# Tani843/Mixed_Precision_Multigrid_Solvers_for_PDEs

Measured on AMD Instinct MI355X. Metric: MDoF/s per V-cycle on 2D Poisson, higher is better.
Workload: dtype f64 (adaptive policy); 1 GPU; 2D Poisson 4097^2 adaptive fp32->fp64 (switch_threshold=1e-6), V(2,2) weighted-Jacobi omega=0.8, 11 levels, 1xMI355X; levels=11, cycle=V(2,2), smoother=jacobi, parallelism=1 GPU

## Files before the change

mixed_precision_multigrid_solvers_for_pdes_amd/csrc/mg_host.hpp:

```cpp
#pragma once

#include <hip/hip_runtime.h>

#include <cmath>
#include <cstdlib>
#include <string>
#include <vector>

#include "../../include/mghip.h"
#include "mg_kernels.hpp"

namespace mgh {

inline size_t esize(int dt) { return dt == MG_F32 ? 4 : 8; }
inline bool valid_dtype(int dt) { return dt == MG_F32 || dt == MG_F64; }

struct Coef {
  double ihx2, ihy2, diag, invD;
  bool pow2;
  bool all_pow2;
};
inline Coef coefs(double hx, double hy, double sigma = 0.0) {
  Coef c;
  c.ihx2 = 1.0 / (hx * hx);
// ... 54 lines not shown
  int* h_int = nullptr;
  mg::HostMailbox* mbox = nullptr;
  mg::HostMailbox* mbox_dev = nullptr;
  unsigned long long mbox_seq = 0;
  void* staging = nullptr;
  int grid_dtype = MG_F64;
  int phase = MG_F64;
  bool promoted = false;
  double fp32_floor = 0.0;
  int switch_reason = 0;
  bool have_rhs = false;
  bool varcoef = false;
  double sigma = 0.0;
  double rd_sigma = -1.0;
  double ring_sumsq[2] = {0, 0};
  unsigned rhs_gen = 1;
  unsigned rings_gen[2] = {0, 0};
  bool iterate_zero = false;
  unsigned zero_norm_gen[2] = {0, 0};
  double zero_norm_val[2] = {0, 0};
  int norm_partials = 0;
  int tail_start = -1;
  bool span_ring[2] = {false, false};
  int tail2_start = -1;
  int tail2_ntop = 0;
  int* d_tail_ops = nullptr;
  int tail_nops = 0;
  bool tail_direct = false;
  double tail_minv[81] = {0};
  double* d_minv = nullptr;
  int minv_n = 0;
  double tail_minv_sigma = -1.0;
  std::string err;
  std::vector<double> adapt_hist;

  int L() const { return (int)lv.size(); }
  int level_dtype_in(int l, int ph) const {
    if (l == L() - 1) return grid_dtype;
    switch (cfg.precision) {
      case MG_PREC_SINGLE: return MG_F32;
      case MG_PREC_SINGLE_MANAGED: return MG_F32;
      case MG_PREC_DEFECT: return MG_F32;
      case MG_PREC_MIXED_LEVELS: return (l >= (cfg.mixed_split > 0 ? cfg.mixed_split : L() / 2)) ? MG_F32 : MG_F64;
      case MG_PREC_ADAPTIVE: return ph;
      default: return MG_F64;
    }
// ... 17 lines not shown
```

mixed_precision_multigrid_solvers_for_pdes_amd/csrc/mg_kernels.hpp:

```cpp
#pragma once

#include <hip/hip_runtime.h>
#include <stdint.h>
#include <type_traits>

namespace mg {

constexpr int kBlock = 256;
constexpr int kTileRowBytes = 512;
constexpr int kTI = 32;
constexpr int kNumXcd = 8;
constexpr int kCoarseTag = 0, kFineTag = 1;
constexpr int kSmJacobi = 0, kSmRbgs = 1;
__host__ __device__ constexpr int sweep_halo(int sm) { return sm == kSmRbgs ? 2 : 1; }

template <typename T> struct VecW { static constexpr int N = 16 / sizeof(T); };

template <typename T> struct alignas(16) Pack {
  T v[VecW<T>::N];
};

template <typename T> __device__ __forceinline__ Pack<T> ldg(const T* p) {
  return *reinterpret_cast<const Pack<T>*>(p);
}
// ... 166 lines not shown
  }
  {
    const int lo = __double2loint(x), hi = __double2hiint(x);
    x += __hiloint2double(__builtin_amdgcn_permlane16_swap(hi, hi, false, false)[1],
                          __builtin_amdgcn_permlane16_swap(lo, lo, false, false)[1]);
  }
  x += dpp_row_move<0x108>(x);
  x += dpp_row_move<0x104>(x);
  x += dpp_row_move<0x102>(x);
  x += dpp_row_move<0x101>(x);
  return x;
}
__device__ __forceinline__ double row0_reduce_sum(double x) {
  x += dpp_row_move<0x108>(x);
  x += dpp_row_move<0x104>(x);
  x += dpp_row_move<0x102>(x);
  x += dpp_row_move<0x101>(x);
  return x;
}
__device__ __forceinline__ double wave_first(double x) {
  return __hiloint2double(__builtin_amdgcn_readfirstlane(__double2hiint(x)), __builtin_amdgcn_readfirstlane(__double2loint(x)));
}

template <int NW = kBlock / 64>
__device__ __forceinline__ double block_reduce_sum(double x, double* red) {
  x = wave_reduce_sum(x);
  const int lane = threadIdx.x & 63, wid = threadIdx.x >> 6;
  if (lane == 0) red[wid] = x;
  __syncthreads();
  double t = 0.0;
  if (threadIdx.x == 0) {
#pragma unroll
    for (int w = 0; w < NW; ++w) t += red[w];
  }
  return t;
}

template <typename T, bool WRITE_R, bool NORM, int TAG>
__global__ __launch_bounds__(kBlock) void residual_kernel(const T* __restrict__ u, const T* __restrict__ rhs,
                                                          T* __restrict__ r, double* __restrict__ partials, TileGeom g,
                                                          T ihx2, T ihy2, T diag, T coeff) {
  using S = TileShape<T>;
  __shared__ __attribute__((aligned(16))) T s[S::LDS_ELEMS];
  __shared__ double red[kBlock / 64];
  const int L = xcd_remap(blockIdx.x, g.ntiles);
  const int ti = L / g.tiles_j, tj = L - ti * g.tiles_j;
  const int i0 = g.i_org + ti * kTI, j0 = tj * S::TJ;
  const int cg = threadIdx.x % S::CG, rg = threadIdx.x / S::CG;
  const int gj0 = j0 + cg * S::N;
  const int lr = rg * S::RPT;

  Pack<T> f[S::RPT];
// ... 1536 lines not shown
```

mixed_precision_multigrid_solvers_for_pdes_amd/csrc/mg_rb_kernels.hpp:

```cpp
#pragma once

#include "mg_kernels.hpp"

namespace mg {

#ifndef MG_RB_HL_MIN
#define MG_RB_HL_MIN 4
#endif
template <typename T, int HALO, int W, int RPT> struct RbShape {
  static constexpr int N = VecW<T>::N;
  static constexpr int HL = (MG_RB_HL_MIN <= 2 && 2 * N >= HALO) ? 2 : ((HALO + N - 1) / N > 4 ? (HALO + N - 1) / N : 4);
  static constexpr int RI = W * RPT;
  static constexpr int RJ = 64 * N;
  static constexpr int TI = RI - 2 * HALO;
  static constexpr int TJ = (64 - 2 * HL) * N;
  static_assert(TI > 0 && TI % 2 == 0, "tile height must be even (coarse rows sit on every other tile row)");
  static_assert(RPT % 2 == 0, "rows per wave must be even (row parities are compile-time constants per strip row)");
  static_assert(HL * N >= HALO, "lateral halo too narrow");
};

#ifndef MG_RB_NT_MODE
#define MG_RB_NT_MODE 3
#endif
template <typename T> __device__ __forceinline__ T dpp_from_lower_lane(T x);
// ... 49 lines not shown
    const f2 sx0 = f2{dn.v[0], dn.v[1]} + f2{up.v[0], up.v[1]}, sx1 = f2{dn.v[2], dn.v[3]} + f2{up.v[2], up.v[3]};
    const f2 sy0 = f2{mid.v[1], mid.v[2]} + f2{left, mid.v[0]}, sy1 = f2{mid.v[3], right} + f2{mid.v[1], mid.v[2]};
    const f2 nb0 = ihx2 * sx0 + ihy2 * sy0, nb1 = ihx2 * sx1 + ihy2 * sy1;
    const f2 t0 = f2{f.v[0], f.v[1]} + nb0, t1 = f2{f.v[2], f.v[3]} + nb1;
    const f2 un0 = use_div ? t0 / D : t0 * invD, un1 = use_div ? t1 / D : t1 * invD;
    const f2 r0 = one_m_omega * m0 + omega * un0, r1 = one_m_omega * m1 + omega * un1;
    Pack<float> res;
    res.v[0] = r0.x; res.v[1] = r0.y; res.v[2] = r1.x; res.v[3] = r1.y;
    return res;
  }
  static __device__ __forceinline__ Pack<float> resid(const Pack<float>& mid, const Pack<float>& dn, const Pack<float>& up, float left,
                                                      float right, const Pack<float>& f, float ihx2, float ihy2, float D, float coeff) {
    const f2 m0 = {mid.v[0], mid.v[1]}, m1 = {mid.v[2], mid.v[3]};
    const f2 sx0 = f2{dn.v[0], dn.v[1]} + f2{up.v[0], up.v[1]}, sx1 = f2{dn.v[2], dn.v[3]} + f2{up.v[2], up.v[3]};
    const f2 sy0 = f2{mid.v[1], mid.v[2]} + f2{left, mid.v[0]}, sy1 = f2{mid.v[3], right} + f2{mid.v[1], mid.v[2]};
    const f2 au0 = coeff * ((sx0 * ihx2 + sy0 * ihy2) - m0 * D), au1 = coeff * ((sx1 * ihx2 + sy1 * ihy2) - m1 * D);
    const f2 r0 = f2{f.v[0], f.v[1]} - au0, r1 = f2{f.v[2], f.v[3]} - au1;
    Pack<float> r;
    r.v[0] = r0.x; r.v[1] = r0.y; r.v[2] = r1.x; r.v[3] = r1.y;
    return r;
  }
};

template <typename T, int W>
__device__ __forceinline__ void rb_exchange(Pack<T>* __restrict__ xb, int w, int lane, const Pack<T>& top, const Pack<T>& bottom,
                                            Pack<T>& above, Pack<T>& below) {
  xb[(w * 2 + 0) * 64 + lane] = top;
  xb[(w * 2 + 1) * 64 + lane] = bottom;
  __syncthreads();
  above = (w > 0) ? xb[((w - 1) * 2 + 1) * 64 + lane] : zero_pack<T>();
  below = (w < W - 1) ? xb[((w + 1) * 2 + 0) * 64 + lane] : zero_pack<T>();
}

template <typename T, int HALO, bool PROLONG, int POST, bool ZERO_INIT, typename TX, typename TC, int SM, int W, int RPT, bool INT, int NT,
          bool VAR, int SPAN = 0>
__device__ __forceinline__ void rb_leg_body(const T* __restrict__ u, const T* __restrict__ rhs, T* __restrict__ out,
                                            const TX* __restrict__ e_coarse, TX* __restrict__ rhs_coarse,
                                            double* __restrict__ partials, const FusedArgs& a, T ihx2, T ihy2, T invD, T D, T omega,
                                            T one_m_omega, T coeff, Pack<T>* __restrict__ xbuf, TX* __restrict__ patch,
                                            double* __restrict__ red, int i0, int j0, const T* __restrict__ acoef, T sigma,
                                            const T* __restrict__ rdiag, T* __restrict__ out2 = nullptr) {
  static_assert(SPAN == 0 || (PROLONG && POST == kPostRestrict && !ZERO_INIT), "a spanning leg is an up leg followed by a down leg");
  using S = RbShape<T, HALO, W, RPT>;
  constexpr int N = S::N;
  constexpr int PH = S::RI / 2 + 2, PW = S::RJ / 2 + 2;
  constexpr int kRowPar = (1 - HALO) & 1;
  const int ri0 = i0 - HALO, rj0 = j0 - S::HL * N;
  const int lane = threadIdx.x & 63, w = __builtin_amdgcn_readfirstlane(threadIdx.x >> 6);
  const int gj0 = rj0 + lane * N;
  const int r_base = w * RPT;
  const bool col_in = INT || (gj0 >= 0 && gj0 < a.nyv);

  const int pic0 = (ri0 >> 1) + a.ci_off, pjc0 = (rj0 >> 1) + a.cj_off;
  if (PROLONG) {
    for (int idx = threadIdx.x; idx < PH * PW; idx += W * 64) {
      const int pr = idx / PW, pc = idx - pr * PW;
      const int ic = pic0 + pr, jc = pjc0 + pc;
      patch[idx] = (INT || (ic >= 0 && ic < a.nxc && jc >= 0 && jc < a.nyc)) ? e_coarse[(size_t)ic * a.ldc + jc] : TX(0);
    }
  }
  Pack<T> F[RPT], U[RPT];
#pragma unroll
  for (int k = 0; k < RPT; ++k) {
    const int gi = ri0 + r_base + k;
    F[k] = zero_pack<T>();
    U[k] = zero_pack<T>();
    if (INT || (gi >= 0 && gi < a.nx && col_in)) {
      F[k] = (NT & 4) ? ldg_nt(rhs + (size_t)gi * a.ld + gj0) : ldg(rhs + (size_t)gi * a.ld + gj0);
      if (!ZERO_INIT) U[k] = (NT & 2) ? ldg_nt(u + (size_t)gi * a.ld + gj0) : ldg(u + (size_t)gi * a.ld + gj0);
    }
  }
  constexpr int AVK = VAR ? RPT + 1 : 1, AHK = VAR ? RPT : 1, AHN = VAR ? N + 1 : 1;
  Pack<T> av[AVK];
  T ah[AHK][AHN];
  Pack<T> RD[AHK];
  if (VAR) {
    Pack<T> A[RPT];
#pragma unroll
    for (int k = 0; k < RPT; ++k) {
      const int gi = ri0 + r_base + k;
      A[k] = zero_pack<T>();
      RD[VAR ? k : 0] = zero_pack<T>();
      if (INT || (gi >= 0 && gi < a.nx && col_in)) {
        A[k] = ldg(acoef + (size_t)gi * a.ld + gj0);
        RD[VAR ? k : 0] = ldg(rdiag + (size_t)gi * a.ld + gj0);
      }
    }
    Pack<T> a_above, a_below;
    rb_exchange<T, W>(xbuf + (size_t)W * 2 * 64, w, lane, A[0], A[RPT - 1], a_above, a_below);
#pragma unroll
    for (int k = 0; k < RPT; ++k) {
      const Pack<T> up = (k > 0) ? A[k > 0 ? k - 1 : 0] : a_above;
      const Pack<T> dn = (k < RPT - 1) ? A[k < RPT - 1 ? k + 1 : 0] : a_below;
      const T left = dpp_from_lower_lane<T>(A[k].v[N - 1]);
      const T right = dpp_from_upper_lane<T>(A[k].v[0]);
#pragma unroll
      for (int e = 0; e < N; ++e) {
        av[VAR ? k : 0].v[e] = T(0.5) * (A[k].v[e] + up.v[e]);
        if (k == RPT - 1) av[VAR ? RPT : 0].v[e] = T(0.5) * (A[k].v[e] + dn.v[e]);
        ah[VAR ? k : 0][VAR ? e : 0] = T(0.5) * (A[k].v[e] + ((e == 0) ? left : A[k].v[e > 0 ? e - 1 : 0]));
      }
      ah[VAR ? k : 0][VAR ? N : 0] = T(0.5) * (A[k].v[N - 1] + right);
    }
  }
  if (PROLONG) {
    __syncthreads();
    using TS = typename std::conditional<(sizeof(TC) > sizeof(T)), TC, T>::type;
    if (INT) {
      constexpr int M = N / 2 + 1;
      const TX* pl = patch + (r_base / 2) * PW + lane * (N / 2);
#pragma unroll
      for (int k = 0; k < RPT; ++k) {
        const bool iodd = ((kRowPar + k) & 1) != 0;
        const int pr = (k + kRowPar) >> 1;
        TC av[M], bv[M];
#pragma unroll
        for (int m = 0; m < M; ++m) {
          av[m] = (TC)pl[pr * PW + m];
          bv[m] = iodd ? (TC)pl[(pr + 1) * PW + m] : TC(0);
        }
#pragma unroll
        for (int e = 0; e < N; ++e) {
          const int m = e >> 1;
          TC val;
          if ((e & 1) == 0) val = iodd ? TC(0.5) * (av[m] + bv[m]) : av[m];
          else val = iodd ? TC(0.25) * (((av[m] + av[m + 1]) + bv[m]) + bv[m + 1]) : TC(0.5) * (av[m] + av[m + 1]);
          U[k].v[e] = (T)((TS)U[k].v[e] + (TS)val);
        }
      }
    } else {
      const TX* pe = patch - ((ptrdiff_t)pic0 * PW + pjc0);
#pragma unroll
      for (int k = 0; k < RPT; ++k) {
        const int gi = ri0 + r_base + k;
        if (gi >= 0 && gi < a.nx && col_in) {
          TC val[N];
          bool ok[N];
          prolong_vec<TX, TC, N>(pe, PW, a.nxc, a.nyc, gi, gj0, a.nx, a.ny, a.sides, val, ok, a.ci_off, a.cj_off);
#pragma unroll
          for (int e = 0; e < N; ++e)
            if (ok[e]) U[k].v[e] = (T)((TS)U[k].v[e] + (TS)val[e]);
        }
      }
    }
  }

  int stage = 0;
  auto run_sweeps = [&](int nsw) {
  const int npass = (SM == kSmRbgs) ? 2 * nsw : nsw;
  for (int s = 0; s < npass; ++s, ++stage) {
    Pack<T> above, below;
    rb_exchange<T, W>(xbuf + (size_t)(stage & 1) * W * 2 * 64, w, lane, U[0], U[RPT - 1], above, below);
    const int colour = s & 1;
    static_assert(N % 2 == 0 && RPT % 2 == 0, "strip rows / lane cells must be even for a workgroup-uniform colour parity");
    const int par0 = (ri0 + rj0 + a.colour_offset) & 1;
    auto pass = [&](auto qp) {
      constexpr int QP = decltype(qp)::value;
      Pack<T> prev = above;
#pragma unroll
      for (int k = 0; k < RPT; ++k) {
        const int r = r_base + k, gi = ri0 + r;
        const Pack<T> mid = U[k];
        const Pack<T> dn = (k < RPT - 1) ? U[k + 1] : below;
        const T left = dpp_from_lower_lane<T>(mid.v[N - 1]);
        const T right = dpp_from_upper_lane<T>(mid.v[0]);
        Pack<T> o = mid;
        const bool row_ok = INT ? ((k > 0 || w > 0) && (k < RPT - 1 || w < W - 1))
                                : (r >= 1 && r < S::RI - 1 && gi >= 1 && gi < a.nx - 1);
        if (row_ok && !VAR) {
          const Pack<T> res = RowMath<T, N>::relax(mid, dn, prev, left, right, F[k], ihx2, ihy2, invD, D, omega, one_m_omega, a.use_div != 0);
#pragma unroll
          for (int e = 0; e < N; ++e) {
            const int gj = gj0 + e;
            const bool mine = (SM != kSmRbgs) || (((QP + k + e) & 1) == 0);
            if ((INT || (gj >= 1 && gj < a.ny - 1)) && mine) o.v[e] = res.v[e];
// ... 22 lines not shown
    else pass(std::integral_constant<int, 0>{});
  }
  };
  run_sweeps(a.nsweep);

  const bool lane_in_tile = lane >= S::HL && lane < 64 - S::HL;
  auto store_tile = [&](T* __restrict__ dst) {
#pragma unroll
    for (int k = 0; k < RPT; ++k) {
      const int r = r_base + k, gi = ri0 + r;
      if (r >= HALO && r < HALO + S::TI && lane_in_tile && (INT || (gi < a.nx && gj0 < a.nyv))) {
        if (NT & 1) stg_nt(dst + (size_t)gi * a.ld + gj0, U[k]); else stg(dst + (size_t)gi * a.ld + gj0, U[k]);
      }
    }
  };
  if (SPAN != 2) store_tile(out);
  if (POST == kPostNone) return;

  Pack<T> R[RPT];
  double acc = 0.0;
  auto residual = [&](auto norm_stage) {
    constexpr bool NORM = decltype(norm_stage)::value;
    Pack<T> above, below;
    rb_exchange<T, W>(xbuf + (size_t)(stage & 1) * W * 2 * 64, w, lane, U[0], U[RPT - 1], above, below);
    ++stage;
#pragma unroll
    for (int k = 0; k < RPT; ++k) {
      const int r = r_base + k, gi = ri0 + r;
      const Pack<T> up = (k > 0) ? U[k - 1] : above;
      const Pack<T> mid = U[k];
      const Pack<T> dn = (k < RPT - 1) ? U[k + 1] : below;
      const T left = dpp_from_lower_lane<T>(mid.v[N - 1]);
      const T right = dpp_from_upper_lane<T>(mid.v[0]);
      Pack<T> o = F[k];
      const bool in_tile = r >= HALO && r < HALO + S::TI && lane_in_tile;
      const bool wanted = !NORM || in_tile;
      const bool row_ok = INT ? ((k > 0 || w > 0) && (k < RPT - 1 || w < W - 1))
                              : (r >= 1 && r < S::RI - 1 && gi >= 1 && gi < a.nx - 1);
      if (wanted && row_ok && !VAR) {
        const Pack<T> rr = RowMath<T, N>::resid(mid, dn, up, left, right, F[k], ihx2, ihy2, D, coeff);
#pragma unroll
        for (int e = 0; e < N; ++e) {
          const int gj = gj0 + e;
          if (INT || (gj >= 1 && gj < a.ny - 1)) {
            o.v[e] = rr.v[e];
            if (NORM && in_tile && (INT || (gi >= a.ni_lo && gi < a.ni_hi && gj >= a.nj_lo && gj < a.nj_hi)))
              acc += (double)o.v[e] * (double)o.v[e];
// ... 8 lines not shown
          T au;
          if (VAR) {
            const T aip = av[VAR ? k + 1 : 0].v[e], aim = av[VAR ? k : 0].v[e];
            const T ajp = ah[VAR ? k : 0][VAR ? e + 1 : 0], ajm = ah[VAR ? k : 0][VAR ? e : 0];
            const T sx = aip * dn.v[e] + aim * up.v[e], sy = ajp * ea + ajm * wv;
            const T D0 = (aip + aim) * ihx2 + (ajp + ajm) * ihy2;
            au = coeff * ((sx * ihx2 + sy * ihy2) - mid.v[e] * ((sigma != T(0)) ? D0 + sigma : D0));
          } else {
            au = coeff * (((dn.v[e] + up.v[e]) * ihx2 + (ea + wv) * ihy2) - mid.v[e] * D);
          }
          const int gj = gj0 + e;
          if (INT || (gj >= 1 && gj < a.ny - 1)) {
            o.v[e] = F[k].v[e] - au;
            if (NORM && in_tile && (INT || (gi >= a.ni_lo && gi < a.ni_hi && gj >= a.nj_lo && gj < a.nj_hi)))
              acc += (double)o.v[e] * (double)o.v[e];
          }
        }
      }
      R[k] = o;
    }
  };
  if (POST == kPostNorm || SPAN) {
    residual(std::true_type{});
    const double t = block_reduce_sum<W>(acc, red);
    if (threadIdx.x == 0) partials[blockIdx.x] = t;
    if (!SPAN) return;
  }
  if (SPAN) {
    run_sweeps(a.nsweep2);
    store_tile(out2);
  }
  residual(std::false_type{});

  {
    Pack<T> above, below;
    rb_exchange<T, W>(xbuf + (size_t)(stage & 1) * W * 2 * 64, w, lane, R[0], R[RPT - 1], above, below);
#pragma unroll
    for (int k = 0; k < RPT; ++k) {
      const int r = r_base + k, fi = ri0 + r;
      const Pack<T> up = (k > 0) ? R[k - 1] : above;
      const Pack<T> mid = R[k];
      const Pack<T> dn = (k < RPT - 1) ? R[k + 1] : below;
      if (((kRowPar + k) & 1) != 0) continue;
      const T nw0 = dpp_from_lower_lane<T>(up.v[N - 1]), w0 = dpp_from_lower_lane<T>(mid.v[N - 1]), sw0 = dpp_from_lower_lane<T>(dn.v[N - 1]);
      if (r < HALO || r >= HALO + S::TI || !lane_in_tile) continue;
      const int ic = (fi >> 1) + a.ci_off;
      if (!INT && (ic < 1 || ic > a.nxc - 2 || fi < 1 || fi > a.nx - 2)) continue;
#pragma unroll
      for (int e = 0; e < N; e += 2) {
        const int fj = gj0 + e, jc = (fj >> 1) + a.cj_off;
        if (!INT && (jc < 1 || jc > a.nyc - 2 || fj < 1 || fj > a.ny - 2)) continue;
        const T NWv = (e == 0) ? nw0 : up.v[e > 0 ? e - 1 : 0], Wv = (e == 0) ? w0 : mid.v[e > 0 ? e - 1 : 0],
                SWv = (e == 0) ? sw0 : dn.v[e > 0 ? e - 1 : 0];
        const T corners = ((NWv + up.v[e + 1]) + SWv) + dn.v[e + 1];
        const T edges = ((up.v[e] + dn.v[e]) + Wv) + mid.v[e + 1];
        rhs_coarse[(size_t)ic * a.ldc + jc] = (TX)((T(1.0 / 16.0) * corners + T(1.0 / 8.0) * edges) + T(1.0 / 4.0) * mid.v[e]);
      }
    }
  }
// ... 32 lines not shown
      if (POST == kPostNorm && threadIdx.x == 0) partials[blockIdx.x] = 0.0;
      return;
    }
  }
  bool interior = !(a.exp_flags & 4) && ri0 >= 1 && ri0 + S::RI <= a.nx - 1 && rj0 >= 1 && rj0 + S::RJ <= a.ny - 1;
  if (PROLONG) {
    const int pic0 = (ri0 >> 1) + a.ci_off, pjc0 = (rj0 >> 1) + a.cj_off;
    interior = interior && pic0 >= 0 && pic0 + PH <= a.nxc && pjc0 >= 0 && pjc0 + PW <= a.nyc;
  }
  if (POST == kPostNorm) interior = interior && i0 >= a.ni_lo && i0 + S::TI <= a.ni_hi && j0 >= a.nj_lo && j0 + S::TJ <= a.nj_hi;
  if (POST == kPostRestrict)
    interior = interior && ((i0 + 1) >> 1) + a.ci_off >= 1 && ((i0 + S::TI - 1) >> 1) + a.ci_off <= a.nxc - 2 &&
               (j0 >> 1) + a.cj_off >= 1 && ((j0 + S::TJ - 2) >> 1) + a.cj_off <= a.nyc - 2;
  if (interior)
    rb_leg_body<T, HALO, PROLONG, POST, ZERO_INIT, TX, TC, SM, W, RPT, true, kNT, VAR>(u, rhs, out, e_coarse, rhs_coarse, partials, a, ihx2, ihy2,
                                                                                invD, D, omega, one_m_omega, coeff, xbuf, patch, red, i0, j0,
                                                                                acoef, sigma, rdiag);
  else
    rb_leg_body<T, HALO, PROLONG, POST, ZERO_INIT, TX, TC, SM, W, RPT, false, kNT, VAR>(u, rhs, out, e_coarse, rhs_coarse, partials, a, ihx2, ihy2,
                                                                                 invD, D, omega, one_m_omega, coeff, xbuf, patch, red, i0, j0,
                                                                                 acoef, sigma, rdiag);
}

template <typename T, int HALO, typename TX, typename TC, int TAG, int SM, int W, int RPT, int SPAN>
__global__ __launch_bounds__(W * 64, 4) void rb_span_kernel(
    const T* __restrict__ u, const T* __restrict__ rhs, T* __restrict__ out_mid, T* __restrict__ out_next,
    const TX* __restrict__ e_coarse, TX* __restrict__ rhs_coarse, double* __restrict__ partials,
    FusedArgs a, T ihx2, T ihy2, T invD, T D, T omega, T one_m_omega, T coeff) {
  using S = RbShape<T, HALO, W, RPT>;
  constexpr int N = S::N;
  constexpr int kNT = (TAG == 2) ? MG_RB_NT_MODE : 0;
  constexpr int PH = S::RI / 2 + 2, PW = S::RJ / 2 + 2;
  constexpr size_t kXBytes = (size_t)2 * W * 2 * 64 * sizeof(Pack<T>);
  constexpr size_t kPatchBytes = (size_t)PH * PW * sizeof(TX);
  __shared__ __attribute__((aligned(16))) unsigned char lds[kXBytes + kPatchBytes];
  __shared__ double red[W];
  Pack<T>* const xbuf = reinterpret_cast<Pack<T>*>(lds);
  TX* const patch = reinterpret_cast<TX*>(lds + kXBytes);

  const int L = xcd_remap(blockIdx.x, a.ntiles);
  const int tiles_i = a.ntiles / a.tiles_j;
  const int per_band = a.band * a.tiles_j;
  const int b = L / per_band, within = L - b * per_band;
  const int rows = min(a.band, tiles_i - b * a.band);
  const int tj = within / rows, ti = b * a.band + (within - tj * rows);
  const int i0 = 1 + ti * S::TI, j0 = tj * S::TJ;
  const int ri0 = i0 - HALO, rj0 = j0 - S::HL * N;
  bool interior = ri0 >= 1 && ri0 + S::RI <= a.nx - 1 && rj0 >= 1 && rj0 + S::RJ <= a.ny - 1;
  {
    const int pic0 = (ri0 >> 1) + a.ci_off, pjc0 = (rj0 >> 1) + a.cj_off;
    interior = interior && pic0 >= 0 && pic0 + PH <= a.nxc && pjc0 >= 0 && pjc0 + PW <= a.nyc;
  }
  interior = interior && i0 >= a.ni_lo && i0 + S::TI <= a.ni_hi && j0 >= a.nj_lo && j0 + S::TJ <= a.nj_hi;
  interior = interior && ((i0 + 1) >> 1) + a.ci_off >= 1 && ((i0 + S::TI - 1) >> 1) + a.ci_off <= a.nxc - 2 &&
             (j0 >> 1) + a.cj_off >= 1 && ((j0 + S::TJ - 2) >> 1) + a.cj_off <= a.nyc - 2;
  if (interior)
    rb_leg_body<T, HALO, true, kPostRestrict, false, TX, TC, SM, W, RPT, true, kNT, false, SPAN>(
        u, rhs, out_mid, e_coarse, rhs_coarse, partials, a, ihx2, ihy2, invD, D, omega, one_m_omega, coeff, xbuf, patch, red, i0, j0,
        nullptr, T(0), nullptr, out_next);
  else
    rb_leg_body<T, HALO, true, kPostRestrict, false, TX, TC, SM, W, RPT, false, kNT, false, SPAN>(
        u, rhs, out_mid, e_coarse, rhs_coarse, partials, a, ihx2, ihy2, invD, D, omega, one_m_omega, coeff, xbuf, patch, red, i0, j0,
        nullptr, T(0), nullptr, out_next);
}

}
```

mixed_precision_multigrid_solvers_for_pdes_amd/csrc/mghip.hip:

```cpp
#include "mg_host.hpp"
#include "mg_kernels.hpp"
#include "mg_rb_kernels.hpp"

#include <hip/hip_runtime.h>

#include <algorithm>
#include <atomic>
#include <chrono>
#include <cmath>
#include <cstdio>
#include <cstdlib>
#include <cstring>
#include <string>
#include <vector>

#include "../../include/mghip.h"

using namespace mgh;

namespace {

thread_local std::string g_last_error;

double now_s() {
// ... 282 lines not shown
  a.ntiles = tiles_i * a.tiles_j;
  a.nsweep = nsweep; a.nsweep2 = 0; a.band = 1; a.use_div = use_div ? 1 : 0; a.colour_offset = poff & 1;
  a.nxc = nxc; a.nyc = nyc; a.ldc = ldc;
  a.ci_off = a.cj_off = 0; a.sides = mg::kAllSides;
  a.ni_lo = 1; a.ni_hi = nx - 1; a.nj_lo = 1; a.nj_hi = ny - 1;
  a.select = 0; a.in_i_lo = a.in_j_lo = 0; a.in_i_hi = a.in_j_hi = 0;
  static const int flags = exp_env("MG_EXP_FLAGS", 0);
  a.exp_flags = flags;
  return a;
}

struct LegGeom {
  int nx, ny, ld, nxc, nyc, ldc;
  double hx, hy, omega, coeff;
  int nsweep, poff;
  bool fine;
  int ci_off = 0, cj_off = 0, sides = mg::kAllSides;
  int ni_lo = -1, ni_hi = -1, nj_lo = -1, nj_hi = -1;
  int select = 0, in_i_lo = 0, in_i_hi = 0, in_j_lo = 0, in_j_hi = 0;
  double sigma = 0.0;
  const void* acoef = nullptr;
  const void* rdiag = nullptr;
  int rb = 0;
};
inline void apply_sub(mg::FusedArgs& a, const LegGeom& g) {
  a.ci_off = g.ci_off; a.cj_off = g.cj_off; a.sides = g.sides;
  if (g.ni_lo >= 0) { a.ni_lo = g.ni_lo; a.ni_hi = g.ni_hi; a.nj_lo = g.nj_lo; a.nj_hi = g.nj_hi; }
  a.select = g.select; a.in_i_lo = g.in_i_lo; a.in_i_hi = g.in_i_hi; a.in_j_lo = g.in_j_lo; a.in_j_hi = g.in_j_hi;
}

inline bool small_tiles(const LegGeom& g, int sm = mg::kSmJacobi) {
  return (long long)g.nx * g.ny <= 1100LL * 1100LL || (g.acoef && sm == mg::kSmRbgs);
}
inline bool tiny_tiles(const LegGeom& g) {
  static const long long lim = exp_env("MG_EXP_TINY", 520);
  return lim > 0 && (long long)g.nx * g.ny <= lim * lim;
}

template <typename T, typename TX, int SM, int TI>
void launch_down_ti(const void* u, const void* rhs, void* out, void* rhs_c, const LegGeom& g, bool zero_init, hipStream_t st) {
  constexpr int HALO = 2 * mg::sweep_halo(SM) + 2;
  const Coef c = coefs(g.hx, g.hy, g.sigma);
  mg::FusedArgs a = fused_args<T, HALO, TI>(g.nx, g.ny, g.ld, g.nsweep, !c.pow2, g.nxc, g.nyc, g.ldc, g.poff);
  apply_sub(a, g);
  void (*k)(const T*, const T*, T*, const TX*, TX*, double*, mg::FusedArgs, T, T, T, T, T, T, T, const T*, T, const T*);
  if (g.acoef) {
// ... 135 lines not shown
  const mg::FusedArgs a = rb_args<T, HALO, W, RPT>(g, !c.pow2);
  const bool nt = rb_stream(g, sizeof(T));
  auto k = MG_RB_PICK(nt, T, HALO, false, mg::kPostNone, false, T, T);
  hipLaunchKernelGGL(k, dim3(a.ntiles), dim3(W * 64), 0, st,
                     (const T*)u, (const T*)rhs, (T*)out, (const T*)nullptr, (T*)nullptr, (double*)nullptr, a, (T)c.ihx2, (T)c.ihy2, (T)c.invD,
                     (T)c.diag, (T)g.omega, (T)(1.0 - g.omega), (T)0, (const T*)g.acoef, (T)g.sigma, (const T*)g.rdiag);
}
template <typename T, typename TX, int SM>
void launch_down_rb(const void* u, const void* rhs, void* out, void* rhs_c, const LegGeom& g, bool zero_init, hipStream_t st) {
  if (g.acoef) launch_down_rb_s<T, TX, SM, MG_EXP_VAR_W, 4, true>(u, rhs, out, rhs_c, g, zero_init, st);
  else launch_down_rb_s<T, TX, SM, MG_EXP_RB_W, 8, false>(u, rhs, out, rhs_c, g, zero_init, st);
}
template <typename T, typename TX, typename TC, int SM>
int launch_up_rb(const void* u, const void* rhs, void* out, const void* e_c, double* partials, const LegGeom& g, bool norm, hipStream_t st) {
  return g.acoef ? launch_up_rb_s<T, TX, TC, SM, MG_EXP_VAR_W, 4, true>(u, rhs, out, e_c, partials, g, norm, st)
                 : launch_up_rb_s<T, TX, TC, SM, MG_EXP_RB_W, 8, false>(u, rhs, out, e_c, partials, g, norm, st);
}
template <typename T, int SM>
void launch_sweeps_rb(const void* u, const void* rhs, void* out, const LegGeom& g, hipStream_t st) {
  if (g.acoef) launch_sweeps_rb_s<T, SM, MG_EXP_VAR_W, 4, true>(u, rhs, out, g, st);
  else launch_sweeps_rb_s<T, SM, MG_EXP_RB_W, 8, false>(u, rhs, out, g, st);
}

template <typename T, typename TX, typename TC, int SM>
int launch_span_rb(const void* u, const void* rhs, void* out_mid, void* out_next, const void* e_c, void* rhs_c, double* partials,
                   const LegGeom& g, int nsweep_pre, hipStream_t st) {
  constexpr int W = 8, RPT = 8;
  constexpr int HALO = 4 * mg::sweep_halo(SM) + 2;
  const Coef c = coefs(g.hx, g.hy, g.sigma);
  mg::FusedArgs a = rb_args<T, HALO, W, RPT>(g, !c.pow2);
  a.nsweep2 = nsweep_pre;
  static const int band = std::max(1, exp_env("MG_EXP_SPAN_BAND", 4));
  a.band = band;
  const bool nt = rb_stream(g, sizeof(T));
  auto k = out_mid ? (nt ? mg::rb_span_kernel<T, HALO, TX, TC, 2, SM, W, RPT, 1> : mg::rb_span_kernel<T, HALO, TX, TC, 1, SM, W, RPT, 1>)
                   : (nt ? mg::rb_span_kernel<T, HALO, TX, TC, 2, SM, W, RPT, 2> : mg::rb_span_kernel<T, HALO, TX, TC, 1, SM, W, RPT, 2>);
  hipLaunchKernelGGL(k, dim3(a.ntiles), dim3(W * 64), 0, st, (const T*)u, (const T*)rhs, (T*)out_mid, (T*)out_next, (const TX*)e_c,
                     (TX*)rhs_c, partials, a, (T)c.ihx2, (T)c.ihy2, (T)c.invD, (T)c.diag, (T)g.omega, (T)(1.0 - g.omega), (T)g.coeff);
  return a.ntiles;
}
template <int SM>
int d_span_sm(int dt, int dcomp, const void* u, const void* rhs, void* out_mid, void* out_next, const void* e_c, void* rhs_c,
              double* partials, const LegGeom& g, int nsweep_pre, hipStream_t st) {
  if (dt == MG_F64 && dcomp == MG_F64) return launch_span_rb<double, double, double, SM>(u, rhs, out_mid, out_next, e_c, rhs_c, partials, g, nsweep_pre, st);
  if (dt == MG_F32 && dcomp == MG_F64) return launch_span_rb<float, float, double, SM>(u, rhs, out_mid, out_next, e_c, rhs_c, partials, g, nsweep_pre, st);
  if (dt == MG_F32 && dcomp == MG_F32) return launch_span_rb<float, float, float, SM>(u, rhs, out_mid, out_next, e_c, rhs_c, partials, g, nsweep_pre, st);
  return -1;
}
int d_span(int dt, int dcomp, const void* u, const void* rhs, void* out_mid, void* out_next, const void* e_c, void* rhs_c,
           double* partials, const LegGeom& g, int nsweep_pre, hipStream_t st, int sm = MG_JACOBI) {
  return sm == MG_RBGS ? d_span_sm<mg::kSmRbgs>(dt, dcomp, u, rhs, out_mid, out_next, e_c, rhs_c, partials, g, nsweep_pre, st)
                       : d_span_sm<mg::kSmJacobi>(dt, dcomp, u, rhs, out_mid, out_next, e_c, rhs_c, partials, g, nsweep_pre, st);
}

bool jacobi_rb(int dt, const void* u, const void* rhs, void* out, int nx, int ny, int ld, double hx, double hy, double omega,
               hipStream_t st, double sigma) {
  static const int on = exp_env("MG_JACOBI_RB", 1);
// ... 495 lines not shown
  LegGeom g{f.nx, f.ny, 0, 0, 0, 0, f.hx, f.hy, 0, 0, 0, 0, true};
  g.rb = rb_mode(h);
  if (!use_rb(g, mg::kSmJacobi)) return false;
  return h->level_dtype(0) == h->level_dtype(1) && (h->level_dtype(0) == MG_F32 || h->grid_dtype == MG_F64);
}
int cycle_span(mg_handle* h, bool keep_mid) {
  const int L = h->L();
  Level& f = h->lv[0];
  Level& c = h->lv[1];
  const int dt = h->level_dtype(0), dc = h->level_dtype(1);
  if (!f.s[dt]) {
    const int rc = alloc_zero(&h->err, &f.s[dt], (size_t)f.nx * f.ld[dt] * esize(dt), h->stream);
    if (rc != MG_OK) return rc;
    h->span_ring[dt] = false;
  }
  if (!h->span_ring[dt]) {
    d_convert_ring(dt, dt, f.u[dt], f.s[dt], f.nx, f.ny, f.ld[dt], f.ld[dt], h->stream);
    h->span_ring[dt] = true;
  }
  LegGeom g{f.nx, f.ny, f.ld[dt], c.nx, c.ny, c.ld[dc], f.hx, f.hy, h->cfg.omega, h->cfg.coeff, 0, h->cfg.colour_offset, true};
  g.sigma = h->sigma;
  g.rb = rb_mode(h);
  g.nsweep = h->cfg.post;
  const int n = d_span(dt, h->grid_dtype, f.u[dt], f.rhs[dt], keep_mid ? f.t[dt] : nullptr, f.s[dt], c.u[dc], c.rhs[dc], h->partials, g,
                       h->cfg.pre, h->stream, h->cfg.smoother);
  if (n < 0) return MG_ERR_INVALID_VALUE;
  void* consumed = f.u[dt];
  f.u[dt] = f.s[dt];
  f.s[dt] = consumed;
  h->norm_partials = n;
  return MG_OK;
}
int cycle_below_fine(mg_handle* h) {
  const int L = h->L();
  int reps = 1;
  if (h->cfg.cycle == MG_CYCLE_W) reps = 2;
  else if (h->cfg.cycle == MG_CYCLE_F) reps = std::max(1, 1 << std::max(0, L - 2));
  for (int k = 0; k < reps; ++k) {
    const int rc = cycle_fused(h, 1, k == 0);
    if (rc != MG_OK) return rc;
  }
  return MG_OK;
}

int fmg_init(mg_handle* h, int ncyc) {
  h->iterate_zero = false;
// ... 361 lines not shown
  return MG_OK;
}

int mg_create(const mg_config* cfg, mg_handle** out) {
  if (!cfg || !out) return fail(nullptr, MG_ERR_INVALID_VALUE, "mg_create: NULL argument");
  *out = nullptr;
  if (cfg->nx < 3 || cfg->ny < 3)
    return fail(nullptr, MG_ERR_INVALID_VALUE, "Grid must have at least 3 points in each direction");
  if (cfg->cycle < MG_CYCLE_V || cfg->cycle > MG_CYCLE_F) return fail(nullptr, MG_ERR_INVALID_VALUE, "unknown cycle type");
  if (cfg->smoother < MG_JACOBI || cfg->smoother > MG_LEXGS) return fail(nullptr, MG_ERR_INVALID_VALUE, "unknown smoother");
  if (cfg->precision < MG_PREC_DOUBLE || cfg->precision > MG_PREC_DEFECT) return fail(nullptr, MG_ERR_INVALID_VALUE, "unknown precision policy");
  if (cfg->pre < 0 || cfg->post < 0 || cfg->max_levels < 1 || cfg->coarse_maxit < 1)
    return fail(nullptr, MG_ERR_INVALID_VALUE, "negative sweep count / max_levels < 1 / coarse_maxit < 1");
  if (!(cfg->x1 > cfg->x0) || !(cfg->y1 > cfg->y0)) return fail(nullptr, MG_ERR_INVALID_VALUE, "empty domain");

  int ndev = 0;
  int rc = mg_device_count(&ndev);
  if (rc != MG_OK) return rc;
  if (ndev <= 0 || cfg->device < 0 || cfg->device >= ndev) return fail(nullptr, MG_ERR_NO_DEVICE, "no such HIP device");
  HIPC(nullptr, hipSetDevice(cfg->device));

  mg_handle* h = new mg_handle();
  h->cfg = *cfg;
  h->grid_dtype = (cfg->precision == MG_PREC_SINGLE) ? MG_F32 : MG_F64;
  h->phase = MG_F64;
  int nx = cfg->nx, ny = cfg->ny;
  for (int level = 0; level < cfg->max_levels; ++level) {
    if (level > 0) {
      if ((nx - 1) % 2 != 0 || (ny - 1) % 2 != 0) break;
      const int cx = (nx - 1) / 2 + 1, cy = (ny - 1) / 2 + 1;
      if (cx < 5 || cy < 5) break;
      nx = cx; ny = cy;
    }
    Level l;
    l.nx = nx; l.ny = ny;
    l.hx = (cfg->x1 - cfg->x0) / (nx - 1);
    l.hy = (cfg->y1 - cfg->y0) / (ny - 1);
    l.ld[0] = pitch_elems(MG_F32, ny);
    l.ld[1] = pitch_elems(MG_F64, ny);
    h->lv.push_back(l);
  }
  auto bail = [&](int code) { release(h); std::string m = h->err; delete h; g_last_error = m; return code; };
  if (hipStreamCreateWithFlags(&h->own_stream, hipStreamNonBlocking) != hipSuccess) { h->err = "hipStreamCreate failed"; return bail(MG_ERR_HIP); }
  h->stream = h->own_stream;
  for (int l = 0; l < h->L(); ++l) {
    Level& v = h->lv[l];
// ... 900 lines not shown
```

Baseline: 78520 MDoF/s.

## Add persistent pipelined spanning-leg kernel with LDS-DMA prefetch of next tile

Adds a persistent Jacobi spanning-leg kernel that launches one workgroup per CU. Each workgroup loops over tiles and prefetches the next tile's rhs and coarse-correction patch into LDS via global_load_lds while the current tile computes. Barriers inside this kernel are replaced with raw s_waitcnt lgkmcnt + s_barrier, avoiding the vmcnt wait that __syncthreads implies. The goal is to hide global-load latency and per-tile launch/ramp overhead. The costs are extra LDS use, a single-occupancy launch bound, and enabling only when speculate==3.

```diff
diff --git a/mixed_precision_multigrid_solvers_for_pdes_amd/csrc/mg_host.hpp b/mixed_precision_multigrid_solvers_for_pdes_amd/csrc/mg_host.hpp
--- a/mixed_precision_multigrid_solvers_for_pdes_amd/csrc/mg_host.hpp
+++ b/mixed_precision_multigrid_solvers_for_pdes_amd/csrc/mg_host.hpp
@@ -100,6 +100,7 @@
   int norm_partials = 0;
   int tail_start = -1;
   bool span_ring[2] = {false, false};
+  int span_wgs = 0;
   int tail2_start = -1;
   int tail2_ntop = 0;
   int* d_tail_ops = nullptr;
diff --git a/mixed_precision_multigrid_solvers_for_pdes_amd/csrc/mg_kernels.hpp b/mixed_precision_multigrid_solvers_for_pdes_amd/csrc/mg_kernels.hpp
--- a/mixed_precision_multigrid_solvers_for_pdes_amd/csrc/mg_kernels.hpp
+++ b/mixed_precision_multigrid_solvers_for_pdes_amd/csrc/mg_kernels.hpp
@@ -212,12 +212,18 @@
   return __hiloint2double(__builtin_amdgcn_readfirstlane(__double2hiint(x)), __builtin_amdgcn_readfirstlane(__double2loint(x)));
 }
 
-template <int NW = kBlock / 64>
+template <bool RAW = false>
+__device__ __forceinline__ void block_sync() {
+  if (RAW) asm volatile("s_waitcnt lgkmcnt(0)\n\ts_barrier" ::: "memory");
+  else __syncthreads();
+}
+
+template <int NW = kBlock / 64, bool RAW = false>
 __device__ __forceinline__ double block_reduce_sum(double x, double* red) {
   x = wave_reduce_sum(x);
   const int lane = threadIdx.x & 63, wid = threadIdx.x >> 6;
   if (lane == 0) red[wid] = x;
-  __syncthreads();
+  block_sync<RAW>();
   double t = 0.0;
   if (threadIdx.x == 0) {
 #pragma unroll
diff --git a/mixed_precision_multigrid_solvers_for_pdes_amd/csrc/mg_rb_kernels.hpp b/mixed_precision_multigrid_solvers_for_pdes_amd/csrc/mg_rb_kernels.hpp
--- a/mixed_precision_multigrid_solvers_for_pdes_amd/csrc/mg_rb_kernels.hpp
+++ b/mixed_precision_multigrid_solvers_for_pdes_amd/csrc/mg_rb_kernels.hpp
@@ -95,25 +95,42 @@
   }
 };
 
-template <typename T, int W>
+template <typename T, int W, bool RAW = false>
 __device__ __forceinline__ void rb_exchange(Pack<T>* __restrict__ xb, int w, int lane, const Pack<T>& top, const Pack<T>& bottom,
                                             Pack<T>& above, Pack<T>& below) {
   xb[(w * 2 + 0) * 64 + lane] = top;
   xb[(w * 2 + 1) * 64 + lane] = bottom;
-  __syncthreads();
+  block_sync<RAW>();
   above = (w > 0) ? xb[((w - 1) * 2 + 1) * 64 + lane] : zero_pack<T>();
   below = (w < W - 1) ? xb[((w + 1) * 2 + 0) * 64 + lane] : zero_pack<T>();
 }
 
+struct RbLoadGlobal {
+  static constexpr bool kStaged = false;
+  __device__ int part() const { return blockIdx.x; }
+  __device__ void after_patch() const {}
+};
+template <typename T, int RPT, class Pf> struct RbStaged {
+  static constexpr bool kStaged = true;
+  const Pack<T> (&F)[RPT];
+  const Pack<T> (&U)[RPT];
+  const Pf& prefetch;
+  int blk;
+  __device__ int part() const { return blk; }
+  __device__ void after_patch() const { prefetch(); }
+};
+
 template <typename T, int HALO, bool PROLONG, int POST, bool ZERO_INIT, typename TX, typename TC, int SM, int W, int RPT, bool INT, int NT,
-          bool VAR, int SPAN = 0>
+          bool VAR, int SPAN = 0, class In = RbLoadGlobal>
 __device__ __forceinline__ void rb_leg_body(const T* __restrict__ u, const T* __restrict__ rhs, T* __restrict__ out,
                                             const TX* __restrict__ e_coarse, TX* __restrict__ rhs_coarse,
                                             double* __restrict__ partials, const FusedArgs& a, T ihx2, T ihy2, T invD, T D, T omega,
                                             T one_m_omega, T coeff, Pack<T>* __restrict__ xbuf, TX* __restrict__ patch,
                                             double* __restrict__ red, int i0, int j0, const T* __restrict__ acoef, T sigma,
-                                            const T* __restrict__ rdiag, T* __restrict__ out2 = nullptr) {
+                                            const T* __restrict__ rdiag, T* __restrict__ out2 = nullptr, const In& in = In()) {
   static_assert(SPAN == 0 || (PROLONG && POST == kPostRestrict && !ZERO_INIT), "a spanning leg is an up leg followed by a down leg");
+  constexpr bool STG = In::kStaged;
+  static_assert(!STG || (SPAN && !VAR), "staged inputs: the pipelined spanning leg only");
   using S = RbShape<T, HALO, W, RPT>;
   constexpr int N = S::N;
   constexpr int PH = S::RI / 2 + 2, PW = S::RJ / 2 + 2;
@@ -125,7 +142,7 @@
   const bool col_in = INT || (gj0 >= 0 && gj0 < a.nyv);
 
   const int pic0 = (ri0 >> 1) + a.ci_off, pjc0 = (rj0 >> 1) + a.cj_off;
-  if (PROLONG) {
+  if (PROLONG && !STG) {
     for (int idx = threadIdx.x; idx < PH * PW; idx += W * 64) {
       const int pr = idx / PW, pc = idx - pr * PW;
       const int ic = pic0 + pr, jc = pjc0 + pc;
@@ -133,14 +150,22 @@
     }
   }
   Pack<T> F[RPT], U[RPT];
-#pragma unroll
-  for (int k = 0; k < RPT; ++k) {
-    const int gi = ri0 + r_base + k;
-    F[k] = zero_pack<T>();
-    U[k] = zero_pack<T>();
-    if (INT || (gi >= 0 && gi < a.nx && col_in)) {
-      F[k] = (NT & 4) ? ldg_nt(rhs + (size_t)gi * a.ld + gj0) : ldg(rhs + (size_t)gi * a.ld + gj0);
-      if (!ZERO_INIT) U[k] = (NT & 2) ? ldg_nt(u + (size_t)gi * a.ld + gj0) : ldg(u + (size_t)gi * a.ld + gj0);
+  if constexpr (STG) {
+#pragma unroll
+    for (int k = 0; k < RPT; ++k) {
+      F[k] = in.F[k];
+      U[k] = in.U[k];
+    }
+  } else {
+#pragma unroll
+    for (int k = 0; k < RPT; ++k) {
+      const int gi = ri0 + r_base + k;
+      F[k] = zero_pack<T>();
+      U[k] = zero_pack<T>();
+      if (INT || (gi >= 0 && gi < a.nx && col_in)) {
+        F[k] = (NT & 4) ? ldg_nt(rhs + (size_t)gi * a.ld + gj0) : ldg(rhs + (size_t)gi * a.ld + gj0);
+        if (!ZERO_INIT) U[k] = (NT & 2) ? ldg_nt(u + (size_t)gi * a.ld + gj0) : ldg(u + (size_t)gi * a.ld + gj0);
+      }
     }
   }
   constexpr int AVK = VAR ? RPT + 1 : 1, AHK = VAR ? RPT : 1, AHN = VAR ? N + 1 : 1;
@@ -177,7 +202,8 @@
     }
   }
   if (PROLONG) {
-    __syncthreads();
+    block_sync<STG>();
+    in.after_patch();
     using TS = typename std::conditional<(sizeof(TC) > sizeof(T)), TC, T>::type;
     if (INT) {
       constexpr int M = N / 2 + 1;
@@ -223,7 +249,7 @@
   const int npass = (SM == kSmRbgs) ? 2 * nsw : nsw;
   for (int s = 0; s < npass; ++s, ++stage) {
     Pack<T> above, below;
-    rb_exchange<T, W>(xbuf + (size_t)(stage & 1) * W * 2 * 64, w, lane, U[0], U[RPT - 1], above, below);
+    rb_exchange<T, W, STG>(xbuf + (size_t)(stage & 1) * W * 2 * 64, w, lane, U[0], U[RPT - 1], above, below);
     const int colour = s & 1;
     static_assert(N % 2 == 0 && RPT % 2 == 0, "strip rows / lane cells must be even for a workgroup-uniform colour parity");
     const int par0 = (ri0 + rj0 + a.colour_offset) & 1;
@@ -292,7 +318,7 @@
   auto residual = [&](auto norm_stage) {
     constexpr bool NORM = decltype(norm_stage)::value;
     Pack<T> above, below;
-    rb_exchange<T, W>(xbuf + (size_t)(stage & 1) * W * 2 * 64, w, lane, U[0], U[RPT - 1], above, below);
+    rb_exchange<T, W, STG>(xbuf + (size_t)(stage & 1) * W * 2 * 64, w, lane, U[0], U[RPT - 1], above, below);
     ++stage;
 #pragma unroll
     for (int k = 0; k < RPT; ++k) {
@@ -347,8 +373,8 @@
   };
   if (POST == kPostNorm || SPAN) {
     residual(std::true_type{});
-    const double t = block_reduce_sum<W>(acc, red);
-    if (threadIdx.x == 0) partials[blockIdx.x] = t;
+    const double t = block_reduce_sum<W, STG>(acc, red);
+    if (threadIdx.x == 0) partials[in.part()] = t;
     if (!SPAN) return;
   }
   if (SPAN) {
@@ -359,7 +385,7 @@
 
   {
     Pack<T> above, below;
-    rb_exchange<T, W>(xbuf + (size_t)(stage & 1) * W * 2 * 64, w, lane, R[0], R[RPT - 1], above, below);
+    rb_exchange<T, W, STG>(xbuf + (size_t)(stage & 1) * W * 2 * 64, w, lane, R[0], R[RPT - 1], above, below);
 #pragma unroll
     for (int k = 0; k < RPT; ++k) {
       const int r = r_base + k, fi = ri0 + r;
@@ -438,23 +464,16 @@
                                                                                  acoef, sigma, rdiag);
 }
 
-template <typename T, int HALO, typename TX, typename TC, int TAG, int SM, int W, int RPT, int SPAN>
-__global__ __launch_bounds__(W * 64, 4) void rb_span_kernel(
-    const T* __restrict__ u, const T* __restrict__ rhs, T* __restrict__ out_mid, T* __restrict__ out_next,
-    const TX* __restrict__ e_coarse, TX* __restrict__ rhs_coarse, double* __restrict__ partials,
-    FusedArgs a, T ihx2, T ihy2, T invD, T D, T omega, T one_m_omega, T coeff) {
+struct SpanTile {
+  int i0, j0;
+  bool interior;
+};
+template <typename T, int HALO, int W, int RPT>
+__device__ __forceinline__ SpanTile span_tile(const FusedArgs& a, int blk) {
   using S = RbShape<T, HALO, W, RPT>;
   constexpr int N = S::N;
-  constexpr int kNT = (TAG == 2) ? MG_RB_NT_MODE : 0;
   constexpr int PH = S::RI / 2 + 2, PW = S::RJ / 2 + 2;
-  constexpr size_t kXBytes = (size_t)2 * W * 2 * 64 * sizeof(Pack<T>);
-  constexpr size_t kPatchBytes = (size_t)PH * PW * sizeof(TX);
-  __shared__ __attribute__((aligned(16))) unsigned char lds[kXBytes + kPatchBytes];
-  __shared__ double red[W];
-  Pack<T>* const xbuf = reinterpret_cast<Pack<T>*>(lds);
-  TX* const patch = reinterpret_cast<TX*>(lds + kXBytes);
-
-  const int L = xcd_remap(blockIdx.x, a.ntiles);
+  const int L = xcd_remap(blk, a.ntiles);
   const int tiles_i = a.ntiles / a.tiles_j;
   const int per_band = a.band * a.tiles_j;
   const int b = L / per_band, within = L - b * per_band;
@@ -470,14 +489,135 @@
   interior = interior && i0 >= a.ni_lo && i0 + S::TI <= a.ni_hi && j0 >= a.nj_lo && j0 + S::TJ <= a.nj_hi;
   interior = interior && ((i0 + 1) >> 1) + a.ci_off >= 1 && ((i0 + S::TI - 1) >> 1) + a.ci_off <= a.nxc - 2 &&
              (j0 >> 1) + a.cj_off >= 1 && ((j0 + S::TJ - 2) >> 1) + a.cj_off <= a.nyc - 2;
-  if (interior)
+  return SpanTile{i0, j0, interior};
+}
+
+template <typename T, int HALO, typename TX, typename TC, int TAG, int SM, int W, int RPT, int SPAN>
+__global__ __launch_bounds__(W * 64, 4) void rb_span_kernel(
+    const T* __restrict__ u, const T* __restrict__ rhs, T* __restrict__ out_mid, T* __restrict__ out_next,
+    const TX* __restrict__ e_coarse, TX* __restrict__ rhs_coarse, double* __restrict__ partials,
+    FusedArgs a, T ihx2, T ihy2, T invD, T D, T omega, T one_m_omega, T coeff) {
+  using S = RbShape<T, HALO, W, RPT>;
+  constexpr int kNT = (TAG == 2) ? MG_RB_NT_MODE : 0;
+  constexpr int PH = S::RI / 2 + 2, PW = S::RJ / 2 + 2;
+  constexpr size_t kXBytes = (size_t)2 * W * 2 * 64 * sizeof(Pack<T>);
+  constexpr size_t kPatchBytes = (size_t)PH * PW * sizeof(TX);
+  __shared__ __attribute__((aligned(16))) unsigned char lds[kXBytes + kPatchBytes];
+  __shared__ double red[W];
+  Pack<T>* const xbuf = reinterpret_cast<Pack<T>*>(lds);
+  TX* const patch = reinterpret_cast<TX*>(lds + kXBytes);
+
+  const SpanTile t = span_tile<T, HALO, W, RPT>(a, blockIdx.x);
+  if (t.interior)
     rb_leg_body<T, HALO, true, kPostRestrict, false, TX, TC, SM, W, RPT, true, kNT, false, SPAN>(
-        u, rhs, out_mid, e_coarse, rhs_coarse, partials, a, ihx2, ihy2, invD, D, omega, one_m_omega, coeff, xbuf, patch, red, i0, j0,
+        u, rhs, out_mid, e_coarse, rhs_coarse, partials, a, ihx2, ihy2, invD, D, omega, one_m_omega, coeff, xbuf, patch, red, t.i0, t.j0,
         nullptr, T(0), nullptr, out_next);
   else
     rb_leg_body<T, HALO, true, kPostRestrict, false, TX, TC, SM, W, RPT, false, kNT, false, SPAN>(
-        u, rhs, out_mid, e_coarse, rhs_coarse, partials, a, ihx2, ihy2, invD, D, omega, one_m_omega, coeff, xbuf, patch, red, i0, j0,
+        u, rhs, out_mid, e_coarse, rhs_coarse, partials, a, ihx2, ihy2, invD, D, omega, one_m_omega, coeff, xbuf, patch, red, t.i0, t.j0,
         nullptr, T(0), nullptr, out_next);
 }
 
-}
+template <int B>
+__device__ __forceinline__ void glds(const void* src, void* dst) {
+  static_assert(B == 16 || B == 4, "LDS-DMA widths in use: 4 and 16 bytes");
+  if constexpr (B == 16)
+    __builtin_amdgcn_global_load_lds((__attribute__((address_space(1))) void*)src, (__attribute__((address_space(3))) void*)dst, 16, 0, 0);
+  else
+    __builtin_amdgcn_global_load_lds((__attribute__((address_space(1))) void*)src, (__attribute__((address_space(3))) void*)dst, 4, 0, 0);
+}
+
+template <typename T, int HALO, typename TX, typename TC, int TAG, int SM, int W, int RPT, int SPAN, bool PF = true>
+__global__ __launch_bounds__(W * 64, 1) void rb_span_pipe_kernel(
+    const T* __restrict__ u, const T* __restrict__ rhs, T* __restrict__ out_mid, T* __restrict__ out_next,
+    const TX* __restrict__ e_coarse, TX* __restrict__ rhs_coarse, double* __restrict__ partials,
+    FusedArgs a, T ihx2, T ihy2, T invD, T D, T omega, T one_m_omega, T coeff, int stride) {
+  using S = RbShape<T, HALO, W, RPT>;
+  constexpr int N = S::N;
+  constexpr int kNT = (TAG == 2) ? MG_RB_NT_MODE : 0;
+  constexpr int PH = S::RI / 2 + 2, PW = S::RJ / 2 + 2;
+  constexpr int kCB = (PW * sizeof(TX)) % 16 == 0 ? 16 : 4;
+  constexpr int kCE = kCB / (int)sizeof(TX);
+  constexpr int kChunks = PH * PW / kCE, kInstr = (kChunks + 63) / 64;
+  constexpr int kPV = VecW<TX>::N, kPacks = PH * PW / kPV;
+  static_assert(std::is_same<T, TX>::value, "the spanning leg's fine and coarse fields share a dtype");
+  static_assert((PH * PW) % kPV == 0 && PW % kCE == 0, "patch rows must hold whole chunks");
+  static_assert((S::TJ / 2) % kCE == 0 && (S::HL * N / 2) % kCE == 0, "patch chunks must be aligned in the coarse array");
+  __shared__ __attribute__((aligned(16))) Pack<T> xbuf[2 * W * 2 * 64];
+  __shared__ __attribute__((aligned(16))) TX patch[PH * PW];
+  __shared__ double red[W];
+  __shared__ __attribute__((aligned(16))) Pack<T> srhs[S::RI * 64];
+  __shared__ __attribute__((aligned(16))) TX spatch[PH * PW];
+
+  const int lane = threadIdx.x & 63, w = __builtin_amdgcn_readfirstlane(threadIdx.x >> 6);
+  Pack<T> UN[RPT];
+  auto issue = [&](int blk) {
+    const SpanTile t = span_tile<T, HALO, W, RPT>(a, blk);
+    const int ri0 = t.i0 - HALO, rj0 = t.j0 - S::HL * N, gj0 = rj0 + lane * N;
+    const bool col_in = t.interior || (gj0 >= 0 && gj0 < a.nyv);
+#pragma unroll
+    for (int k = 0; k < RPT; ++k) {
+      const int gi = ri0 + w * RPT + k;
+      const bool ok = t.interior || (gi >= 0 && gi < a.nx && col_in);
+      if (ok) glds<16>(rhs + (size_t)gi * a.ld + gj0, srhs + (w * RPT + k) * 64);
+    }
+    const int pic0 = (ri0 >> 1) + a.ci_off, pjc0 = (rj0 >> 1) + a.cj_off;
+    for (int q = w; q < kInstr; q += W) {
+      const int c = q * 64 + lane, pr = (c * kCE) / PW, pc = c * kCE - pr * PW;
+      const int ic = pic0 + pr, jc = pjc0 + pc;
+      if (c < kChunks && (t.interior || (ic >= 0 && ic < a.nxc && jc >= 0 && jc < a.nyc)))
+        glds<kCB>(e_coarse + (size_t)ic * a.ldc + jc, spatch + q * 64 * kCE);
+    }
+#pragma unroll
+    for (int k = 0; k < RPT; ++k) {
+      const int gi = ri0 + w * RPT + k;
+      UN[k] = zero_pack<T>();
+      if (t.interior || (gi >= 0 && gi < a.nx && col_in))
+        UN[k] = (kNT & 2) ? ldg_nt(u + (size_t)gi * a.ld + gj0) : ldg(u + (size_t)gi * a.ld + gj0);
+    }
+  };
+  auto run = [&](auto int_tag, int blk, const SpanTile& t) {
+    constexpr bool INT = decltype(int_tag)::value;
+    const int ri0 = t.i0 - HALO, rj0 = t.j0 - S::HL * N, gj0 = rj0 + lane * N;
+    const int pic0 = (ri0 >> 1) + a.ci_off, pjc0 = (rj0 >> 1) + a.cj_off;
+    for (int p = threadIdx.x; p < kPacks; p += W * 64) {
+      Pack<TX> v = reinterpret_cast<const Pack<TX>*>(spatch)[p];
+      if (!INT) {
+#pragma unroll
+        for (int e = 0; e < kPV; ++e) {
+          const int idx = p * kPV + e, pr = idx / PW, ic = pic0 + pr, jc = pjc0 + (idx - pr * PW);
+          if (!(ic >= 0 && ic < a.nxc && jc >= 0 && jc < a.nyc)) v.v[e] = TX(0);
+        }
+      }
+      reinterpret_cast<Pack<TX>*>(patch)[p] = v;
+    }
+    const bool col_in = INT || (gj0 >= 0 && gj0 < a.nyv);
+    Pack<T> F[RPT], U[RPT];
+#pragma unroll
+    for (int k = 0; k < RPT; ++k) {
+      const int gi = ri0 + w * RPT + k;
+      F[k] = zero_pack<T>();
+      if (INT || (gi >= 0 && gi < a.nx && col_in)) F[k] = srhs[(w * RPT + k) * 64 + lane];
+      U[k] = UN[k];
+    }
+    auto prefetch = [&]() {
+      if (PF && blk + stride < a.ntiles) issue(blk + stride);
+    };
+    const RbStaged<T, RPT, decltype(prefetch)> in{F, U, prefetch, blk};
+    rb_leg_body<T, HALO, true, kPostRestrict, false, TX, TC, SM, W, RPT, INT, kNT, false, SPAN>(
+        u, rhs, out_mid, e_coarse, rhs_coarse, partials, a, ihx2, ihy2, invD, D, omega, one_m_omega, coeff, xbuf, patch, red, t.i0, t.j0,
+        nullptr, T(0), nullptr, out_next, in);
+  };
+
+  if (PF) issue(blockIdx.x);
+  for (int blk = blockIdx.x; blk < a.ntiles; blk += stride) {
+    if (!PF) issue(blk);
+    asm volatile("s_waitcnt vmcnt(0)" ::: "memory");
+    block_sync<true>();
+    const SpanTile t = span_tile<T, HALO, W, RPT>(a, blk);
+    if (t.interior) run(std::true_type{}, blk, t);
+    else run(std::false_type{}, blk, t);
+  }
+}
+
+}
diff --git a/mixed_precision_multigrid_solvers_for_pdes_amd/csrc/mghip.hip b/mixed_precision_multigrid_solvers_for_pdes_amd/csrc/mghip.hip
--- a/mixed_precision_multigrid_solvers_for_pdes_amd/csrc/mghip.hip
+++ b/mixed_precision_multigrid_solvers_for_pdes_amd/csrc/mghip.hip
@@ -328,6 +328,7 @@
   const void* acoef = nullptr;
   const void* rdiag = nullptr;
   int rb = 0;
+  int span_wgs = 0;
 };
 inline void apply_sub(mg::FusedArgs& a, const LegGeom& g) {
   a.ci_off = g.ci_off; a.cj_off = g.cj_off; a.sides = g.sides;
@@ -509,6 +510,12 @@
   else launch_sweeps_rb_s<T, SM, MG_EXP_RB_W, 8, false>(u, rhs, out, g, st);
 }
 
+#ifndef MG_EXP_SPAN_NOPF
+#define MG_EXP_SPAN_NOPF 0
+#endif
+#if MG_EXP_SPAN_NOPF && !defined(MG_EXPERIMENTS)
+#error "MG_EXP_SPAN_NOPF needs -DMG_EXPERIMENTS (a measurement build)"
+#endif
 template <typename T, typename TX, typename TC, int SM>
 int launch_span_rb(const void* u, const void* rhs, void* out_mid, void* out_next, const void* e_c, void* rhs_c, double* partials,
                    const LegGeom& g, int nsweep_pre, hipStream_t st) {
@@ -520,6 +527,15 @@
   static const int band = std::max(1, exp_env("MG_EXP_SPAN_BAND", 4));
   a.band = band;
   const bool nt = rb_stream(g, sizeof(T));
+  if constexpr (SM == mg::kSmJacobi) if (g.span_wgs > 0 && g.ci_off == 0 && g.cj_off == 0 && g.select == 0) {
+    constexpr bool PF = !MG_EXP_SPAN_NOPF;
+    auto k = out_mid ? (nt ? mg::rb_span_pipe_kernel<T, HALO, TX, TC, 2, SM, W, RPT, 1, PF> : mg::rb_span_pipe_kernel<T, HALO, TX, TC, 1, SM, W, RPT, 1, PF>)
+                     : (nt ? mg::rb_span_pipe_kernel<T, HALO, TX, TC, 2, SM, W, RPT, 2, PF> : mg::rb_span_pipe_kernel<T, HALO, TX, TC, 1, SM, W, RPT, 2, PF>);
+    hipLaunchKernelGGL(k, dim3(std::min(g.span_wgs, a.ntiles)), dim3(W * 64), 0, st, (const T*)u, (const T*)rhs, (T*)out_mid, (T*)out_next,
+                       (const TX*)e_c, (TX*)rhs_c, partials, a, (T)c.ihx2, (T)c.ihy2, (T)c.invD, (T)c.diag, (T)g.omega, (T)(1.0 - g.omega),
+                       (T)g.coeff, g.span_wgs);
+    return a.ntiles;
+  }
   auto k = out_mid ? (nt ? mg::rb_span_kernel<T, HALO, TX, TC, 2, SM, W, RPT, 1> : mg::rb_span_kernel<T, HALO, TX, TC, 1, SM, W, RPT, 1>)
                    : (nt ? mg::rb_span_kernel<T, HALO, TX, TC, 2, SM, W, RPT, 2> : mg::rb_span_kernel<T, HALO, TX, TC, 1, SM, W, RPT, 2>);
   hipLaunchKernelGGL(k, dim3(a.ntiles), dim3(W * 64), 0, st, (const T*)u, (const T*)rhs, (T*)out_mid, (T*)out_next, (const TX*)e_c,
@@ -1061,6 +1077,7 @@
   g.sigma = h->sigma;
   g.rb = rb_mode(h);
   g.nsweep = h->cfg.post;
+  g.span_wgs = (h->cfg.speculate == 3) ? h->span_wgs : 0;
   const int n = d_span(dt, h->grid_dtype, f.u[dt], f.rhs[dt], keep_mid ? f.t[dt] : nullptr, f.s[dt], c.u[dc], c.rhs[dc], h->partials, g,
                        h->cfg.pre, h->stream, h->cfg.smoother);
   if (n < 0) return MG_ERR_INVALID_VALUE;
@@ -1468,6 +1485,10 @@
 
   mg_handle* h = new mg_handle();
   h->cfg = *cfg;
+  {
+    int cus = 0;
+    if (hipDeviceGetAttribute(&cus, hipDeviceAttributeMultiprocessorCount, cfg->device) == hipSuccess) h->span_wgs = cus / mg::kNumXcd * mg::kNumXcd;
+  }
   h->grid_dtype = (cfg->precision == MG_PREC_SINGLE) ? MG_F32 : MG_F64;
   h->phase = MG_F64;
   int nx = cfg->nx, ny = cfg->ny;
```

Result: slower. 77710 MDoF/s, median of 2 (-1.0%).
